# anzeA/Tarok

Hardware: AMD Instinct MI355X
Metric: env steps/sec at 65 536 parallel 4-player games; 1/2/4/8 MI355X (higher is better)
Workload: dtype u64

## Files before the change

include/tarok_env.h:

```cpp
#ifndef TAROK_ENV_H
#define TAROK_ENV_H
#include <stdint.h>

#ifdef __cplusplus
extern "C" {
#endif

#define TAROK_ABI_VERSION 5
#define TAROK_MAX_CARDS_PER_LAUNCH 192
#define TAROK_GAMES_AHEAD 14

#define TAROK_OK 0
#define TAROK_EINVAL (-1)
#define TAROK_EHIP (-2)
#define TAROK_ENOMEM (-3)
#define TAROK_ENODEV (-4)

#define TAROK_MIX_ALL 0
#define TAROK_MIX_NAVADNA3 1
#define TAROK_MIX_BOT 2
#define TAROK_MIX_FIXED 16

#define TAROK_DEFER_EXCHANGE 1
#define TAROK_AUTO_RESET 2
// ... 133 lines not shown

int tarok_learn_returns_gae(tarok_env *env, int T, const uint8_t *done, const int16_t *reward, const uint64_t *obs,
                            const float *logp, const float *value, const uint8_t *action, float reward_scale, float gamma,
                            float lambda, float *rec_out, float *stats_out, float *scratch, void *stream);

int tarok_learn_returns_seats(tarok_env *env, int T, const uint8_t *done, const int16_t *reward, const uint64_t *obs,
                              const float *logp, const float *value, const uint8_t *action, float reward_scale, int gae,
                              float gamma, float lambda, int seats, const uint8_t *seats_per_game, float *rec_out,
                              float *stats_out, float *scratch, void *stream);

#define TAROK_LEARN_SELECT_TILE 2048
int64_t tarok_learn_select_scratch_bytes(int64_t M);
int tarok_learn_select(tarok_env *env, int64_t M, const float *rec, int64_t *index_out, int64_t *count_out,
                       void *scratch, void *stream);

int tarok_learn_chain(tarok_env *env, int64_t B, const uint64_t *feature_words, const int64_t *index, const float *rec,
                      const float *stats, float clip, float vf_coef, float ent_coef, const void *w1, const float *b1,
                      const void *w2, const float *b2, const void *w3, const float *b3, const void *w3t, const void *w2t,
                      uint64_t *Xw, void *H1, void *H2, void *dOut, void *dH2, void *dH1, float *scratch, float *terms_out,
                      float *running, void *stream);

int64_t tarok_learn_workspace_bytes(tarok_env *env);
int tarok_learn_dw(tarok_env *env, int64_t B, const uint64_t *Xw, const void *H1,
                   const void *H2, const void *dOut, const void *dH2, const void *dH1, const float *terms,
                   void *workspace, float *grad_out, void *stream);

int tarok_learn_adam(tarok_env *env, float *param, const float *grad, float *m, float *v, int32_t *step, float lr,
                     float beta1, float beta2, float eps, float max_norm, void *w1, void *w2, void *w3, void *w3t,
                     void *w2t, float *gnorm_out, int apply, void *stream);

int tarok_debug_stamps(tarok_env *env, uint64_t *stamps);
int tarok_debug_stamps_sized(tarok_env *env, uint64_t *stamps, int64_t n_words);
int tarok_debug_refill_selftest(tarok_env *env, int kind, int per_slot, uint32_t episode0, int order, int reps, uint64_t *report_out);

int tarok_get_state(tarok_env *env, uint64_t *lanes_out, void *stream);
int tarok_set_state(tarok_env *env, const uint64_t *lanes_in, void *stream);
int tarok_get_counters(tarok_env *env, uint32_t *episode_out, int32_t *score_sum_out, void *stream);

#ifdef __cplusplus
}
#endif
#endif
```

tarok_amd/_native.py:

```python
import ctypes as C
import os
import subprocess

HERE = os.path.dirname(os.path.abspath(__file__))
ROOT = os.path.dirname(HERE)
SRC = os.path.join(HERE, "csrc", "tarok_env.hip")
DEPS = [SRC, os.path.join(HERE, "csrc", "tarok_device.h"), os.path.join(HERE, "csrc", "deal_network.inc"),
        os.path.join(HERE, "csrc", "tarok_learner.inc"),
        os.path.join(ROOT, "include", "tarok_env.h")]
LIB_PATH = os.path.join(HERE, "libtarokenv.so")
ARCH = "gfx950"
COMPILE_FLAGS = ["--offload-arch=" + ARCH, "-O3", "-std=c++17", "-mllvm", "-amdgpu-kernarg-preload-count=16",
                 "-I", os.path.join(ROOT, "include")]

SYMBOLS = [
    "tarok_strerror", "tarok_abi_version", "tarok_device_count", "tarok_last_hip_error",
    "tarok_create", "tarok_destroy", "tarok_num_games", "tarok_set_option", "tarok_reset", "tarok_exchange",
    "tarok_legal_actions", "tarok_step", "tarok_prefetch", "tarok_policy_random", "tarok_step_random",
    "tarok_run_random", "tarok_krog_random", "tarok_rollout_random", "tarok_get_state", "tarok_set_state", "tarok_get_counters", "tarok_debug_stamps", "tarok_debug_stamps_sized", "tarok_debug_refill_selftest", "tarok_observe", "tarok_sample_policy", "tarok_policy_mlp", "tarok_policy_step", "tarok_policy_step_seats", "tarok_policy_step_versus", "tarok_expand_features", "tarok_ppo_loss",
    "tarok_targets_ref", "tarok_learn_returns", "tarok_learn_returns_gae", "tarok_learn_returns_seats", "tarok_learn_select_scratch_bytes", "tarok_learn_select",
    "tarok_learn_chain", "tarok_learn_workspace_bytes", "tarok_learn_dw", "tarok_learn_adam",
    "tarok_observe_ref", "tarok_observe_exchange_ref", "tarok_observe_hands_ref", "tarok_get_history", "tarok_set_history",
]


class TarokNativeError(RuntimeError):
    pass


def hipcc_path():
    for p in (os.environ.get("HIPCC"), "/opt/rocm/bin/hipcc"):
        if p and os.path.exists(p):
            return p
    return "hipcc"


def needs_build():
    if not os.path.exists(LIB_PATH):
        return True
    t = os.path.getmtime(LIB_PATH)
    return any(os.path.getmtime(d) > t for d in DEPS)


def build(force=False, verbose=False):
    if not force and not needs_build():
        return LIB_PATH
    import fcntl
    with open(LIB_PATH + ".lock", "w") as lock:
        fcntl.flock(lock, fcntl.LOCK_EX)
        try:
            if force or needs_build():
                tmp = "%s.tmp.%d" % (LIB_PATH, os.getpid())
# ... 61 lines not shown
    L.tarok_step_random.restype = i32; L.tarok_step_random.argtypes = [vp, vp, vp, vp, vp, vp, i32, vp]
    L.tarok_run_random.restype = i32; L.tarok_run_random.argtypes = [vp, i64, i32, i32, i32, vp, vp, vp, vp, i32, vp]
    L.tarok_krog_random.restype = i32; L.tarok_krog_random.argtypes = [vp, i32, i64, vp, vp, vp, vp, vp, i32, vp]
    L.tarok_rollout_random.restype = i32; L.tarok_rollout_random.argtypes = [vp, u32, vp, vp, vp, vp, vp, vp]
    L.tarok_get_state.restype = i32; L.tarok_get_state.argtypes = [vp, vp, vp]
    L.tarok_observe.restype = i32; L.tarok_observe.argtypes = [vp, vp, vp]
    L.tarok_sample_policy.restype = i32; L.tarok_sample_policy.argtypes = [vp, vp, vp, vp, vp, vp]
    L.tarok_policy_mlp.restype = i32; L.tarok_policy_mlp.argtypes = [vp] * 14
    L.tarok_policy_step.restype = i32; L.tarok_policy_step.argtypes = [vp] * 16 + [i32, vp]
    L.tarok_policy_step_seats.restype = i32; L.tarok_policy_step_seats.argtypes = [vp, i32, vp] + [vp] * 15 + [i32, vp]
    L.tarok_policy_step_versus.restype = i32; L.tarok_policy_step_versus.argtypes = [vp, i32, vp] + [vp] * 21 + [i32, vp]
    L.tarok_expand_features.restype = i32; L.tarok_expand_features.argtypes = [vp, i64, vp, vp, vp, vp]
    f32 = C.c_float
    L.tarok_ppo_loss.restype = i32; L.tarok_ppo_loss.argtypes = [vp, i64] + [vp] * 7 + [f32] * 3 + [vp] * 4
    L.tarok_targets_ref.restype = i32; L.tarok_targets_ref.argtypes = [vp, i32] + [vp] * 6 + [f32] + [vp] * 3
    L.tarok_learn_returns.restype = i32; L.tarok_learn_returns.argtypes = [vp, i32] + [vp] * 6 + [f32] + [vp] * 4
    L.tarok_learn_returns_gae.restype = i32; L.tarok_learn_returns_gae.argtypes = [vp, i32] + [vp] * 6 + [f32] * 3 + [vp] * 4
    L.tarok_learn_returns_seats.restype = i32
    L.tarok_learn_returns_seats.argtypes = [vp, i32] + [vp] * 6 + [f32, i32, f32, f32, i32] + [vp] * 5
    L.tarok_learn_select_scratch_bytes.restype = i64; L.tarok_learn_select_scratch_bytes.argtypes = [i64]
    L.tarok_learn_select.restype = i32; L.tarok_learn_select.argtypes = [vp, i64] + [vp] * 5
    L.tarok_learn_chain.restype = i32; L.tarok_learn_chain.argtypes = [vp, i64] + [vp] * 4 + [f32] * 3 + [vp] * 18
    L.tarok_learn_workspace_bytes.restype = i64; L.tarok_learn_workspace_bytes.argtypes = [vp]
    L.tarok_learn_dw.restype = i32; L.tarok_learn_dw.argtypes = [vp, i64] + [vp] * 10
    L.tarok_learn_adam.restype = i32; L.tarok_learn_adam.argtypes = [vp] * 6 + [f32] * 5 + [vp] * 6 + [i32, vp]
    L.tarok_observe_ref.restype = i32; L.tarok_observe_ref.argtypes = [vp, vp, vp, vp]
    L.tarok_observe_exchange_ref.restype = i32; L.tarok_observe_exchange_ref.argtypes = [vp, vp, vp]
    L.tarok_observe_hands_ref.restype = i32; L.tarok_observe_hands_ref.argtypes = [vp, vp, vp]
    L.tarok_get_history.restype = i32; L.tarok_get_history.argtypes = [vp, vp, vp]
    L.tarok_set_history.restype = i32; L.tarok_set_history.argtypes = [vp, vp, vp]
    L.tarok_debug_stamps.restype = i32; L.tarok_debug_stamps.argtypes = [vp, vp]
    L.tarok_debug_stamps_sized.restype = i32; L.tarok_debug_stamps_sized.argtypes = [vp, vp, i64]
    L.tarok_debug_refill_selftest.restype = i32; L.tarok_debug_refill_selftest.argtypes = [vp, i32, i32, u32, i32, i32, vp]
    L.tarok_set_state.restype = i32; L.tarok_set_state.argtypes = [vp, vp, vp]
    L.tarok_get_counters.restype = i32; L.tarok_get_counters.argtypes = [vp, vp, vp, vp]
    _lib = L
    return L


def check(code):
    if code != 0:
        L = lib()
        raise TarokNativeError("libtarokenv: %s (code %d, hipError %d)" % (
            L.tarok_strerror(code).decode(), code, L.tarok_last_hip_error()))
```

tarok_amd/csrc/tarok_device.h:

```cpp
#pragma once
#include <hip/hip_runtime.h>
#include <stdint.h>

typedef unsigned long long u64;
typedef uint32_t u32;

#define TK_VGPR_BUDGET(B) __attribute__((amdgpu_num_vgpr((B) - 1)))
#define TK_KERNEL(threads, B) __global__ __launch_bounds__(threads) TK_VGPR_BUDGET(B)
#define TK_VGPR_STR2(x) #x
#define TK_VGPR_STR(x) TK_VGPR_STR2(x)
#define TK_VGPR_TOP(B, TOP)                                                                                           \
    do {                                                                                                              \
        static_assert((B) % 8 == 0 && (B) <= 256 && (TOP) == (B) - 1, "TK_VGPR_TOP(B, B - 1), B a multiple of 8");     \
        asm volatile("" ::: "v" TK_VGPR_STR(TOP));                                                                    \
    } while (0)

#define TK_BIT(i) (1ULL << (i))
#define TK_DECK ((1ULL << 54) - 1)
#define TK_TAROK (((1ULL << 22) - 1) << 32)
#define TK_PAGAT TK_BIT(32)
#define TK_V5 (TK_BIT(7) | TK_BIT(15) | TK_BIT(23) | TK_BIT(31) | TK_BIT(32) | TK_BIT(52) | TK_BIT(53))
#define TK_V4 (TK_BIT(6) | TK_BIT(14) | TK_BIT(22) | TK_BIT(30))
#define TK_V3 (TK_BIT(5) | TK_BIT(13) | TK_BIT(21) | TK_BIT(29))
#define TK_V2 (TK_BIT(4) | TK_BIT(12) | TK_BIT(20) | TK_BIT(28))
// ... 22 lines not shown
    g.C = x0 & TK_DECK; g.A = y0 & TK_DECK; g.B = y1 & TK_DECK;
    u32 m0 = (u32)(x0 >> 54), m2 = (u32)(y0 >> 54), m3 = (u32)(y1 >> 54);
    g.nt = 0; g.leader = (m0 >> 2) & 3; g.trick_no = (m0 >> 4) & 15; g.phase = m0 >> 8;
    g.talon = x1 & ((1ULL << 36) - 1);
    g.trick = 0;
    g.tl = (u32)(x1 >> 60) & 7; g.error = (u32)(x1 >> 63);
    g.contract = m2 & 15; g.declarer = (m2 >> 4) & 3; g.king = (m2 >> 6) & 3;
    g.team = m3 & 15; g.epar = (m3 >> 4) & 15; g.cprev = 0;
}

__device__ __forceinline__ void pack_play(const Game &g, u64 &x0, u64 &x1) {
    x0 = g.C | ((u64)(g.nt | (g.leader << 2) | (g.trick_no << 4) | (g.phase << 8)) << 54);
    x1 = g.talon | ((u64)g.trick << 36) | ((u64)g.tl << 60) | ((u64)g.error << 63);
}
__device__ __forceinline__ void pack_seats(const Game &g, u64 &y0, u64 &y1) {
    y0 = g.A | ((u64)(g.contract | (g.declarer << 4) | (g.king << 6) | ((g.cprev >> 2) << 8)) << 54);
    y1 = g.B | ((u64)(g.team | (g.epar << 4) | ((g.cprev & 3) << 8)) << 54);
}
__device__ __forceinline__ void pack(const Game &g, u64 &x0, u64 &x1, u64 &y0, u64 &y1) {
    pack_play(g, x0, x1);
    pack_seats(g, y0, y1);
}

__device__ __forceinline__ int popc64(u64 m) { return __popcll(m); }

template <class F> constexpr u32 tk_tt(F f) { return f(0xF0u, 0xCCu, 0xAAu) & 0xFFu; }
#define TK_BITOP3(a, b, c, ...) ((u32)__builtin_amdgcn_bitop3_b32((a), (b), (c), tk_tt([](u32 a_, u32 b_, u32 c_) { return (__VA_ARGS__); })))
#define TK_LO(x) ((u32)(x))
#define TK_HI(x) ((u32)((x) >> 32))
#ifndef TK_KEEP_VGPR
#define TK_KEEP_VGPR(x) asm volatile("" : "+v"(x))
#endif
#define TK_U64(lo, hi) (((u64)(u32)(hi) << 32) | (u64)(u32)(lo))

__device__ __forceinline__ u64 seat_cards(const Game &g, u32 s) {
    u64 a = (s & 1) ? g.A : ~g.A, b = (s & 2) ? g.B : ~g.B;
    return a & b & TK_DECK;
}
#define TK_C_PAD (0xFFC00000ULL << 32)
template <bool C_PADDED = false>
__device__ __forceinline__ u64 hand_of(const Game &g, u32 s) {
    u32 ma = (u32)((int)(s << 31) >> 31), mb = (u32)((int)(s << 30) >> 31);
    u32 tl = TK_BITOP3(TK_LO(g.A), ma, TK_LO(g.C), ~c_ & ~(a_ ^ b_));
    u32 th = TK_BITOP3(TK_HI(g.A), ma, TK_HI(g.C), ~c_ & ~(a_ ^ b_));
    u32 hl = TK_BITOP3(tl, TK_LO(g.B), mb, a_ & ~(b_ ^ c_));
    u32 hh = TK_BITOP3(th, TK_HI(g.B), mb, a_ & ~(b_ ^ c_));
    if (!C_PADDED) hh &= 0x3FFFFFu;
    return TK_U64(hl, hh);
}
template <int S> __device__ __forceinline__ u64 pile_of(const Game &g) {
    u32 l, h;
    if (S == 0)      { l = TK_BITOP3(TK_LO(g.A), TK_LO(g.B), TK_LO(g.C), ~a_ & ~b_ & c_); h = TK_BITOP3(TK_HI(g.A), TK_HI(g.B), TK_HI(g.C), ~a_ & ~b_ & c_); }
    else if (S == 1) { l = TK_BITOP3(TK_LO(g.A), TK_LO(g.B), TK_LO(g.C), a_ & ~b_ & c_);  h = TK_BITOP3(TK_HI(g.A), TK_HI(g.B), TK_HI(g.C), a_ & ~b_ & c_); }
    else if (S == 2) { l = TK_BITOP3(TK_LO(g.A), TK_LO(g.B), TK_LO(g.C), ~a_ & b_ & c_);  h = TK_BITOP3(TK_HI(g.A), TK_HI(g.B), TK_HI(g.C), ~a_ & b_ & c_); }
    else             { l = TK_BITOP3(TK_LO(g.A), TK_LO(g.B), TK_LO(g.C), a_ & b_ & c_);   h = TK_BITOP3(TK_HI(g.A), TK_HI(g.B), TK_HI(g.C), a_ & b_ & c_); }
    return TK_U64(l, h);
}

__device__ __forceinline__ u64 ids_mask(u64 ids, int first, int n) {
    u64 m = 0;
#pragma unroll
    for (int i = 0; i < 6; i++)
        if (i >= first && i < first + n) m |= 1ULL << ((ids >> (6 * i)) & 63);
    return m;
}
__device__ __forceinline__ u64 talon_all(const Game &g) { return ids_mask(g.talon, 0, 6); }
// ... 424 lines not shown
```

tarok_amd/csrc/tarok_env.hip:

```cpp
#include "tarok_device.h"

#include <hip/hip_runtime.h>
#include <stddef.h>
#include <stdint.h>
#include <stdio.h>
#include <stdlib.h>
#include <string.h>
#include <type_traits>
#include <utility>

#include "../../include/tarok_env.h"

#define TK_BLOCK 256
#define TK_PF_SLOTS (4 * TK_BLOCK)
#define TK_GRAPH_CACHE 16
#define TK_REFILL_CAP (TK_BLOCK * TK_AHEAD)
#define TK_REFILL_FAN 8
#define TK_RC(group, k) ((((size_t)(group)) * 4 + (k)) * 32)
#define TK_BULK_EVERY 32u
#define TK_BULK_CAP ((TK_BULK_EVERY / 4) * TK_BLOCK)

#define TK_AHEAD TAROK_GAMES_AHEAD
#define TK_LINE(episode) ((u32)(episode) % (u32)TK_AHEAD)
#define TK_FINQ 128
#define TK_STREAM_STORE(ptr, val) __builtin_nontemporal_store((val), (ptr))
#define TK_WAIT_LOADS() __builtin_amdgcn_s_waitcnt(0x0F70)
#define TK_RARE(c) __builtin_expect(!!(c), 0)
#define TK_USUAL(c) __builtin_expect(!!(c), 1)

struct __attribute__((aligned(64))) AuxLine {
    ulonglong2 n01, n23; u64 nkey; u32 nep;
    u32 pad[5];
};
struct __attribute__((aligned(64))) Aux { AuxLine line[TK_AHEAD]; };
static_assert(sizeof(AuxLine) == 64 && sizeof(Aux) == 64 * TK_AHEAD, "64 bytes per next-game line");
static_assert((TK_BLOCK * sizeof(Aux)) % 128 == 0, "a play group's next-game lines end on an L2 line boundary");
static_assert(TK_AHEAD >= 2 && TK_AHEAD <= 15, "epar / cprev are 4-bit fields");
struct __attribute__((aligned(32))) Counters {
    int4 score_sum;
    u32 episode;
    u32 pad[3];
};
static_assert(sizeof(Counters) == 32, "Counters is half a cache line");

struct tarok_env {
    int device;
    int64_t n;
    u64 offset, seed;
    int mix, flags;
    ulonglong2 *s01, *s23;
    Aux *aux;
    Counters *cnt;
    uint16_t *nstale;
    u64 *gkey;
    uint8_t *hist;
    u64 *rlist;
    u32 *rcount;
    u64 *elist;
    u32 *epoch;
// ... 286 lines not shown
            lists = elist; cap = TK_BULK_CAP;
#pragma unroll
            for (u32 q = 0; q < TK_REFILL_FAN; q++) {
                bool has = q < fan && g0 + q < play_groups;
                cum[q + 1] = cum[q] + (has ? min(tk_ld(&rcount[TK_RC(g0 + q, 2 + which)]), (u32)TK_BULK_CAP) : 0u);
            }
        }
        for (u32 j = tid; j < cum[TK_REFILL_FAN]; j += nthreads) {
            u32 q = 0;
#pragma unroll
            for (u32 r = 1; r < TK_REFILL_FAN; r++) q += j >= cum[r] ? 1u : 0u;
            u32 base = 0;
#pragma unroll
            for (u32 r = 0; r < TK_REFILL_FAN; r++) base = (r == q) ? cum[r] : base;
            u64 en = tk_ld(&lists[((int64_t)(g0 + q) * 2 + which) * cap + (j - base)]);
            deal_into_buffer(aux, (int64_t)(g0 + q) * TK_BLOCK + (u32)(en & 0xFFFF), (u32)(en >> 32), seed, offset, mix);
        }
    }
    if (any || bulk) {
        __syncthreads();
        if (any && tid < fan && g0 + tid < play_groups) rcount[TK_RC(g0 + tid, par ^ 1u)] = 0u;
        if (bulk && tid < fan && g0 + tid < play_groups) rcount[TK_RC(g0 + tid, 2 + which)] = 0u;
    }
}

template <bool HIST>
__device__ __forceinline__ void play_role(
    u32 group, u32 tid,
    int64_t n, u64 seed, u64 offset, int mix, int flags, int cards, int64_t stride, TkCount count, u32 *epoch, u32 play_groups, u32 fan,
    uint8_t *__restrict__ action_out, int16_t *__restrict__ reward,
    uint8_t *__restrict__ done, uint16_t *__restrict__ trick, u64 *__restrict__ obs, uint8_t *__restrict__ hist,
    ulonglong2 *__restrict__ s01, ulonglong2 *__restrict__ s23, Aux *aux, Counters *__restrict__ cnt,
    u64 *__restrict__ gkey, u64 *rlist, u32 *rcount, u64 *__restrict__ stamps) {
    __shared__ unsigned short push_list[TK_REFILL_CAP];
    __shared__ u32 push_ep[TK_BLOCK];
    __shared__ u32 push_count;
    __shared__ u32 finq[TK_BLOCK / 64][9][TK_FINQ];
    __shared__ int sacc[4][TK_BLOCK];
    if (tid == 0) push_count = 0;
    sacc[0][tid] = 0; sacc[1][tid] = 0; sacc[2][tid] = 0; sacc[3][tid] = 0;
    __syncthreads();
    u32 fq_head = 0, fq_n = 0;
    u32 (*fq)[TK_FINQ] = finq[tid >> 6];
    auto drain_finished = [&](u32 cnt_) __attribute__((always_inline)) {
        u32 lane = tid & 63;
        if (lane < cnt_) {
            u32 e = (fq_head + lane) & (TK_FINQ - 1);
            Game f;
            f.A = TK_U64(fq[0][e], fq[1][e]); f.B = TK_U64(fq[2][e], fq[3][e]); f.C = TK_U64(fq[4][e], fq[5][e] & 0x3FFFFFu);
            u32 m = fq[7][e], ri = fq[8][e];
            f.talon = TK_U64(fq[6][e], (m >> 24) & 15u);
            f.contract = m & 15; f.declarer = (m >> 4) & 3; f.king = (m >> 6) & 3; f.team = (m >> 8) & 15;
            f.tl = (m >> 12) & 7; f.trick_no = (m >> 16) & 15; f.leader = (m >> 20) & 3;
            f.trick = 0; f.nt = 0; f.phase = TK_PHASE_DONE; f.error = 0; f.epar = 0; f.cprev = 0;
            u64 sc = final_scores(f);
            u32 t = ri & 0xFFFFu;
            if (reward) {
                u64 rs = sc;
                if ((flags & TAROK_REWARD_REF) && (f.contract == TK_BERAC || f.contract == TK_ODPRTI_BERAC)) {
                    int dv = f.trick_no >= 12 ? -20 : 20;
                    u32 d = f.declarer;
                    rs = pack_scores(d == 0 ? (int)(int16_t)(sc & 0xFFFF) : dv, d == 1 ? (int)(int16_t)((sc >> 16) & 0xFFFF) : dv,
                                     d == 2 ? (int)(int16_t)((sc >> 32) & 0xFFFF) : dv, d == 3 ? (int)(int16_t)(sc >> 48) : dv);
                }
                reinterpret_cast<u64 *>(reward)[(int64_t)group * TK_BLOCK + t + (int64_t)(ri >> 16) * stride] = rs;
            }
            atomicAdd(&sacc[0][t], (int)(int16_t)(sc & 0xFFFF)); atomicAdd(&sacc[1][t], (int)(int16_t)((sc >> 16) & 0xFFFF));
            atomicAdd(&sacc[2][t], (int)(int16_t)((sc >> 32) & 0xFFFF)); atomicAdd(&sacc[3][t], (int)(int16_t)(sc >> 48));
        }
        fq_head = (fq_head + cnt_) & (TK_FINQ - 1);
        fq_n -= cnt_;
    };
    u64 t_real0 = 0, t_cyc0 = 0, t_play = 0;
    if (stamps) { t_real0 = __builtin_amdgcn_s_memrealtime(); t_cyc0 = __builtin_amdgcn_s_memtime(); }
    int64_t i = (int64_t)group * TK_BLOCK + tid;
    bool valid = i < n;
    int64_t ic = valid ? i : n - 1;
    Game g;
    load_game(g, s01, s23, ic);
    u64 key = gkey[ic];
    bool autoreset = (flags & TAROK_AUTO_RESET) != 0;
    bool berac = g.contract == TK_BERAC || g.contract == TK_ODPRTI_BERAC;
    bool spec = valid && ((g.phase == TK_PHASE_PLAY && (int)g.nt + cards >= 4 &&
                           (berac || (int)(g.trick_no * 4 + g.nt) + cards >= 48)) ||
                          g.phase == TK_PHASE_DONE);
    u32 cprev0 = valid ? g.cprev : 0u;
    u32 allowed = TK_AHEAD - min(cprev0, (u32)TK_AHEAD);
    int4 acc = make_int4(0, 0, 0, 0);
    u32 cur_ep = 0;
    ulonglong2 na = make_ulonglong2(0, 0), nb = na, na2 = na, nb2 = na;
    u64 nkey = 0, nkey2 = 0;
    u32 nep1 = 0, nep2 = 0;
    bool ok1 = false, ok2 = false;
    auto line_tag = [&](bool &ok, u32 &nep, u32 tag) __attribute__((always_inline)) { nep = tag; ok = true; };
    static_assert(offsetof(AuxLine, nkey) == 32 && offsetof(AuxLine, nep) == 40, "key and tag share the line's third 16 bytes");
    auto load_line = [&](const AuxLine *ln, ulonglong2 &a, ulonglong2 &b, u64 &k, bool &ok, u32 &nep) __attribute__((always_inline)) {
        a = ln->n01; b = ln->n23;
        uint3 kt = *reinterpret_cast<const uint3 *>(__builtin_assume_aligned(&ln->nkey, 16));
        k = TK_U64(kt.x, kt.y);
        line_tag(ok, nep, kt.z);
    };
    const bool all_play = autoreset && __ballot(valid && g.phase == TK_PHASE_PLAY) == ~0ULL;
    const bool aligned = all_play && (cards & 3) == 0 && __ballot(g.nt != 0) == 0;
    if (spec) {
        acc = cnt[i].score_sum;
        cur_ep = cnt[i].episode;
        if (autoreset && allowed > 0) {
            load_line(&aux[i].line[TK_LINE(g.epar + 1)], na, nb, nkey, ok1, nep1);
            if (!aligned && allowed > 1 && cards > 4)
                load_line(&aux[i].line[TK_LINE(g.epar + 2)], na2, nb2, nkey2, ok2, nep2);
        }
    }
    TK_WAIT_LOADS();
    u32 par = launch_phase<1>(count, play_groups, fan) & 1u;
    launch_counted<1>(epoch);
    g.cprev = 0;
    u32 consumed = 0;
    bool resync = false;
    bool blocked = false;
    bool acc_dirty = false, seats_dirty = false, touched = false;
    u64 legal = (valid && g.phase == TK_PHASE_PLAY) ? legal_now(g) : 0;
    u64 c_lead = 0;
    u32 legal_hi = 0;
    u32 rctr = 0, ocar = 0;
    u32 resync_v = 0;
    u32 lim = spec ? allowed : 0u;
    auto fetch_lines = [&](bool lacks, bool lacks2) __attribute__((always_inline)) {
        if (lacks) load_line(&aux[i].line[TK_LINE(cur_ep + 1)], na, nb, nkey, ok1, nep1);
        if (lacks2) load_line(&aux[i].line[TK_LINE(cur_ep + 2)], na2, nb2, nkey2, ok2, nep2);
    };
    auto play_card = [&](auto all_tag, auto nt_tag, auto std_tag, int64_t row, int ci) __attribute__((always_inline)) {
        constexpr bool ALL = decltype(all_tag)::value;
        constexpr int NT = decltype(nt_tag)::value;
        constexpr bool STD = decltype(std_tag)::value;
        if constexpr (NT >= 0) g.nt = (u32)NT;
        constexpr bool TOP_UP_EARLY = ALL && NT == 0;
        constexpr bool TOP_UP_LATE = !(ALL && NT == 3);
        if constexpr (TOP_UP_EARLY) {
            if (nep1 != cur_ep + 1 && consumed < lim) {
                u32 off = g.epar + 1 >= (u32)TK_AHEAD ? 0u : (g.epar + 1) * (u32)sizeof(AuxLine);
                load_line(reinterpret_cast<const AuxLine *>(reinterpret_cast<const char *>(aux[i].line) + off), na, nb, nkey, ok1, nep1);
            }
        }
        const bool v = ALL ? true : valid;
// ... 109 lines not shown
                        TK_WAIT_LOADS();
                    }
                }
                bool swap = renew && !blocked && ok1 && nep1 == cur_ep + 1;
                if (swap) {
                    swap_in();
                    ok1 = ok2 && consumed + 1 < allowed;
                    ok2 = false;
                }
                bool deal_here = renew && !swap;
                if (deal_here && consumed < allowed) resync = true;
                if (deal_here) blocked = true;
                deal_in_place(deal_here, g, key);
                if (renew) { cur_ep++; consumed++; seats_dirty = true; }
            }
        }
        if constexpr (ALIGNED && NT < 3) legal = legal_mask_follow(hand_of<true>(g, (g.leader + g.nt) & 3), g.trick & 63, g.contract, legal_hi);
        else if constexpr (ALIGNED) legal = legal_mask(hand_of<true>(g, g.leader), false, 0u, g.contract);
        else legal = (ALL || (v && g.phase == TK_PHASE_PLAY)) ? legal_now(g) : 0;
        if (v) {
            const u32 fin01 = ALL ? (u32)res : (fin ? 1u : 0u);
            if constexpr (ALIGNED) {
                if constexpr (NT < 3) ocar += TK_OBS_CARD;
                else ocar = obs_carry(g.leader, g.trick_no << 2);
                TK_STREAM_STORE(&obs[row], obs_word_with(ocar, g.error, fin01, legal));
            } else {
                TK_STREAM_STORE(&obs[row], obs_word_with<true>(g, false, legal) | ((u64)(ALL ? fin01 : ((fin || g.phase == TK_PHASE_DONE) ? 1u : 0u)) << 62));
            }
            if (STD || done) TK_STREAM_STORE(&done[row], (uint8_t)fin01);
        }
    };
    int64_t row = i;
    typedef std::integral_constant<int, -1> nt_any;
    if (all_play) {
        if (aligned) {
            auto tricks = [&](auto std_tag) __attribute__((always_inline)) {
                touched = true; seats_dirty = true;
                g.C |= TK_C_PAD;
                rctr = rng_ctr(128u + g.trick_no * 4).v;
                ocar = obs_carry(g.leader, g.trick_no << 2);
                for (int c = 0; c < cards; c += 4) {
                    play_card(std::true_type{}, std::integral_constant<int, 0>{}, std_tag, row, c); row += stride;
                    play_card(std::true_type{}, std::integral_constant<int, 1>{}, std_tag, row, c + 1); row += stride;
                    play_card(std::true_type{}, std::integral_constant<int, 2>{}, std_tag, row, c + 2); row += stride;
                    play_card(std::true_type{}, std::integral_constant<int, 3>{}, std_tag, row, c + 3); row += stride;
                }
                g.C &= TK_DECK;
            };
            if (action_out && done && !trick) tricks(std::true_type{});
            else tricks(std::false_type{});
        } else {
            for (int c = 0; c < cards; c++, row += stride) play_card(std::true_type{}, nt_any{}, std::false_type{}, row, c);
        }
    } else {
        for (int c = 0; c < cards; c++, row += stride) play_card(std::false_type{}, nt_any{}, std::false_type{}, row, c);
    }
    while (fq_n) drain_finished(min(fq_n, 64u));
    __builtin_amdgcn_s_waitcnt(0xC07F);
    {
        int4 sa = make_int4(sacc[0][tid], sacc[1][tid], sacc[2][tid], sacc[3][tid]);
        if (sa.x | sa.y | sa.z | sa.w) { acc.x += sa.x; acc.y += sa.y; acc.z += sa.z; acc.w += sa.w; acc_dirty = true; }
    }
    u32 np = (resync || resync_v != 0) ? (u32)TK_AHEAD : min(consumed, (u32)TK_AHEAD);
    if (valid) {
        g.cprev = np;
        if (acc_dirty) cnt[i].score_sum = acc;
        if (consumed) { cnt[i].episode = cur_ep; gkey[i] = key; }
        if (touched || consumed || cprev0 != np) store_game(g, s01, s23, i, seats_dirty || cprev0 != np);
    }
    if (stamps) t_play = __builtin_amdgcn_s_memtime() - t_cyc0;
    if (valid && np) {
        u32 pos = atomicAdd(&push_count, np);
        push_ep[tid] = cur_ep;
        for (u32 j = 0; j < np; j++) push_list[pos + j] = (unsigned short)(j * TK_BLOCK + tid);
    }
    __syncthreads();
    u32 total = push_count;
    u64 *lst = rlist + ((int64_t)group * 2 + par) * TK_REFILL_CAP;
    for (u32 j = tid; j < total; j += TK_BLOCK) {
        u32 en = push_list[j], t = en % TK_BLOCK;
        lst[j] = ((u64)(push_ep[t] + TK_AHEAD - en / TK_BLOCK) << 32) | t;
    }
    if (tid == 0) rcount[TK_RC(group, par)] = total;
    if (stamps && (tid & 63) == 0) {
        u64 w = (u64)i >> 6;
        stamps[3 * w + 0] = t_real0;
        stamps[3 * w + 1] = __builtin_amdgcn_s_memrealtime();
        stamps[3 * w + 2] = ((__builtin_amdgcn_s_memtime() - t_cyc0) << 32) | (t_play & 0xFFFFFFFFULL);
    }
}

#define TK_PLAY_ARGS                                                                                                             \
    int64_t n, u64 seed, u64 offset, int mix, int flags, int cards, int64_t stride, u32 play_groups, u32 *epoch, u32 fan,         \
        uint8_t *__restrict__ action_out, int16_t *__restrict__ reward,                                                           \
        uint8_t *__restrict__ done, uint16_t *__restrict__ trick, u64 *__restrict__ obs, uint8_t *__restrict__ hist,              \
        ulonglong2 *__restrict__ s01, ulonglong2 *__restrict__ s23, Aux *aux, Counters *__restrict__ cnt,                         \
        u64 *__restrict__ gkey, u64 *rlist, u32 *rcount, u64 *__restrict__ stamps
template <bool HIST>
TK_KERNEL(TK_BLOCK, 168) __attribute__((amdgpu_waves_per_eu(3, 3))) void k_play_wide(TK_PLAY_ARGS) {
    TK_VGPR_TOP(168, 167);
    TkCount count = launch_count<1>(epoch, play_groups);
    if (blockIdx.x >= play_groups)
        refill_role<false>(blockIdx.x - play_groups, threadIdx.x, TK_BLOCK, seed, offset, mix, play_groups, count, epoch, fan, false, aux, rlist, rcount, nullptr);
    else {
        play_role<HIST>(blockIdx.x, threadIdx.x, n, seed, offset, mix, flags, cards, stride, count, epoch, play_groups, fan,
                        action_out, reward, done, trick, obs, hist, s01, s23, aux, cnt, gkey, rlist, rcount, stamps);
    }
}

__device__ __forceinline__ void deal_in_place_wave(bool deal_here, Game &gd, u64 &kd, u64 seed, u64 offset, int64_t i, u32 ep, int mix) {
    u64 pend = __ballot(deal_here);
    if (pend == 0) return;
    u64 dkey = 0;
    if (deal_here) dkey = game_key(seed, offset + (u64)i, ep);
    u64 h0 = 0, h1 = 0, h2 = 0, h3 = 0, tal = 0;
    u32 lane = __lane_id();
    while (pend) {
        int l = __builtin_ctzll(pend);
        pend &= pend - 1;
        u32 klo = (u32)__builtin_amdgcn_readlane((int)(u32)dkey, l);
        u32 khi = (u32)__builtin_amdgcn_readlane((int)(u32)(dkey >> 32), l);
// ... 1399 lines not shown
    if (!e || !obs_out) return TAROK_EINVAL;
    HIPCHK(hipSetDevice(e->device));
    hipLaunchKernelGGL(k_legal, grid_for(e->n), dim3(TK_BLOCK), 0, (hipStream_t)stream, e->n, e->s01, e->s23,
                       (u64 *)obs_out, seat_out);
    HIPCHK(hipGetLastError());
    return TAROK_OK;
}

static inline u64 *stamps_for(const tarok_env *e, size_t words) { return (e->stamps && e->stamps_words >= words) ? e->stamps : nullptr; }

static inline void launch_play(tarok_env *e, bool random, int cards, int64_t stride, const uint8_t *action_in,
                               uint8_t *action_out, int16_t *reward, uint8_t *done, uint16_t *trick, uint64_t *obs,
                               int flags, hipStream_t s) {
    u32 groups = (u32)((e->n + TK_BLOCK - 1) / TK_BLOCK);
    u32 fan = e->refill_fan;
    dim3 grid(groups + (groups + fan - 1) / fan);
    e->launched = 1;
    if (cards == 1 && e->lazy_refill) grid = dim3(groups);
    if (cards == 1) {
#define TK_LAUNCH_STEP(R, Z)                                                                                             \
    hipLaunchKernelGGL((k_step<R, Z>), grid, dim3(TK_BLOCK), 0, s, e->n, e->seed, e->offset, e->mix, flags, groups, e->epoch, \
                       fan, action_in, action_out, reward, done, trick, (u64 *)obs, e->hist, e->s01, e->s23, e->aux, e->cnt,  \
                       e->gkey, e->rlist, e->rcount, e->elist)
        if (e->lazy_refill) { if (random) TK_LAUNCH_STEP(true, true); else TK_LAUNCH_STEP(false, true); }
        else                { if (random) TK_LAUNCH_STEP(true, false); else TK_LAUNCH_STEP(false, false); }
#undef TK_LAUNCH_STEP
        return;
    }
#define TK_LAUNCH_PLAY(H)                                                                                              \
    hipLaunchKernelGGL((k_play_wide<H>), grid, dim3(TK_BLOCK), 0, s, e->n, e->seed, e->offset, e->mix, flags, cards, stride, \
                       groups, e->epoch, fan, action_out, reward, done, trick, (u64 *)obs, e->hist, e->s01,            \
                       e->s23, e->aux, e->cnt, e->gkey, e->rlist, e->rcount, stamps)
    u64 *stamps = stamps_for(e, 3 * (size_t)((e->n + 63) / 64));
    if (e->hist) TK_LAUNCH_PLAY(true); else TK_LAUNCH_PLAY(false);
#undef TK_LAUNCH_PLAY
}

int tarok_step(tarok_env *e, const uint8_t *action, int16_t *reward_out, uint8_t *done_out, uint16_t *trick_out,
               uint64_t *obs_out, int flags, void *stream) {
    if (!e || !action || !obs_out) return TAROK_EINVAL;
    HIPCHK(hipSetDevice(e->device));
    launch_play(e, false, 1, e->n, action, nullptr, reward_out, done_out, trick_out, obs_out, flags, (hipStream_t)stream);
    HIPCHK(hipGetLastError());
    return TAROK_OK;
}

static inline void launch_policy(tarok_env *e, const uint64_t *obs, uint8_t *action, hipStream_t s) {
    if (e->n >= (1 << 21) && (((uintptr_t)obs & 15) | ((uintptr_t)action & 1)) == 0)
        hipLaunchKernelGGL(k_policy_x4, dim3((unsigned)((e->n + 4 * TK_BLOCK - 1) / (4 * TK_BLOCK))), dim3(TK_BLOCK), 0, s, e->n,
                           (const u64 *)obs, e->gkey, action);
    else
        hipLaunchKernelGGL(k_policy, grid_for(e->n), dim3(TK_BLOCK), 0, s, e->n, (const u64 *)obs, e->gkey, action);
}

int tarok_policy_random(tarok_env *e, const uint64_t *obs, uint8_t *action_out, void *stream) {
    if (!e || !obs || !action_out) return TAROK_EINVAL;
    HIPCHK(hipSetDevice(e->device));
    launch_policy(e, obs, action_out, (hipStream_t)stream);
    HIPCHK(hipGetLastError());
    return TAROK_OK;
}

int tarok_step_random(tarok_env *e, uint8_t *action_out, int16_t *reward_out, uint8_t *done_out, uint16_t *trick_out,
                      uint64_t *obs_out, int flags, void *stream) {
    if (!e || !obs_out) return TAROK_EINVAL;
    HIPCHK(hipSetDevice(e->device));
// ... 102 lines not shown
    void *buf = nullptr;
    unsigned long long *rep = nullptr;
    HIPCHK(hipMalloc(&buf, rows * (size_t)n * (8 + 8 + 1 + 1) + 64));
    hipError_t r = hipMalloc((void **)&rep, 49 * sizeof(unsigned long long));
    if (r == hipSuccess) r = hipMemset(rep, 0, 49 * sizeof(unsigned long long));
    if (r != hipSuccess) { (void)hipFree(buf); g_last_hip = (int)r; return TAROK_EHIP; }
    uint64_t *obs = (uint64_t *)buf;
    int16_t *reward = (int16_t *)(obs + rows * n);
    uint8_t *action = (uint8_t *)(reward + rows * n * 4), *done = action + rows * n;
    u32 groups = (u32)((n + TK_BLOCK - 1) / TK_BLOCK);
    for (int it = 0; it < reps; it++) {
        hipLaunchKernelGGL(k_dbg_clear_lines, grid_for(n), dim3(TK_BLOCK), 0, 0, e->aux, n);
        hipLaunchKernelGGL(k_dbg_fill_lists, dim3(groups), dim3(TK_BLOCK), 0, 0, e->rlist, e->rcount, n, (u32)per_slot, episode0, (u32)order);
        if (kind == 0) launch_play(e, true, 1, n, nullptr, action, reward, done, nullptr, obs, TAROK_AUTO_RESET, 0);
        else if (kind == 1) {
            hipLaunchKernelGGL(k_legal, grid_for(n), dim3(TK_BLOCK), 0, 0, n, e->s01, e->s23, (u64 *)obs, (int8_t *)nullptr);
            launch_policy(e, obs, action, 0);
            launch_play(e, false, 1, n, action, nullptr, reward, done, nullptr, obs, TAROK_AUTO_RESET, 0);
        } else launch_play(e, true, kind == 2 ? 4 : 2, n, nullptr, action, reward, done, nullptr, obs, TAROK_AUTO_RESET, 0);
        hipLaunchKernelGGL(k_dbg_check_lines, grid_for(n), dim3(TK_BLOCK), 0, 0, e->aux, n, e->seed, e->offset, e->mix, (u32)per_slot, episode0, rep);
    }
    r = hipDeviceSynchronize();
    if (r == hipSuccess) r = hipMemcpy(report_out, rep, 49 * sizeof(unsigned long long), hipMemcpyDeviceToHost);
    if (r == hipSuccess) r = hipMemset(e->rcount, 0, TK_RC(groups, 0) * sizeof(u32));
    if (r == hipSuccess) {
        hipLaunchKernelGGL(k_dbg_clear_lines, grid_for(n), dim3(TK_BLOCK), 0, 0, e->aux, n);
        r = hipDeviceSynchronize();
    }
    (void)hipFree(buf); (void)hipFree(rep);
    if (r != hipSuccess) { g_last_hip = (int)r; return TAROK_EHIP; }
    return TAROK_OK;
}

int tarok_observe(tarok_env *e, void *features_out, void *stream) {
    if (!e || !features_out) return TAROK_EINVAL;
    HIPCHK(hipSetDevice(e->device));
    hipLaunchKernelGGL(k_observe, grid_for(e->n), dim3(TK_BLOCK), 0, (hipStream_t)stream, e->n, e->s01, e->s23,
                       (uint2 *)features_out);
    HIPCHK(hipGetLastError());
    return TAROK_OK;
}

int tarok_observe_ref(tarok_env *e, uint8_t *record_out, int32_t *meta_out, void *stream) {
    if (!e || !record_out) return TAROK_EINVAL;
    if (!e->hist) return TAROK_EINVAL;
    HIPCHK(hipSetDevice(e->device));
    hipLaunchKernelGGL(k_observe_ref, dim3((unsigned)((e->n + OR_GAMES - 1) / OR_GAMES)), dim3(256), 0, (hipStream_t)stream, e->n,
                       e->s01, e->s23, e->hist, (uint4 *)record_out, (int4 *)meta_out);
    HIPCHK(hipGetLastError());
    return TAROK_OK;
}

int tarok_observe_exchange_ref(tarok_env *e, uint8_t *out, void *stream) {
    if (!e || !out) return TAROK_EINVAL;
    HIPCHK(hipSetDevice(e->device));
    hipLaunchKernelGGL(k_observe_exchange_ref, grid_for(e->n), dim3(TK_BLOCK), 0, (hipStream_t)stream, e->n, e->s01, e->s23,
                       (uint2 *)out);
    HIPCHK(hipGetLastError());
    return TAROK_OK;
}

int tarok_observe_hands_ref(tarok_env *e, uint8_t *out, void *stream) {
    if (!e || !out) return TAROK_EINVAL;
    HIPCHK(hipSetDevice(e->device));
    hipLaunchKernelGGL(k_observe_hands_ref, grid_for(e->n), dim3(TK_BLOCK), 0, (hipStream_t)stream, e->n, e->s01, e->s23,
                       (uint2 *)out);
// ... 308 lines not shown
```

tarok_amd/env.py:

```python
import ctypes as C

import numpy as np
import torch

from . import _native
from . import karte as K


def _u64(t):
    return t.detach().cpu().numpy().view(np.uint64)


class Obs:

    def __init__(self, words):
        self.words = words

    @property
    def mask(self):
        return self.words & K.OBS_MASK

    @property
    def seat(self):
        return (self.words >> K.OBS_SEAT_SHIFT) & 3
# ... 22 lines not shown
            raise _native.TarokNativeError("TarokVecEnv needs an MI355X: no GPU is visible and there is no CPU fallback")
        self.L = L
        self.n = int(n_games)
        self.device_index = int(device)
        self.device = torch.device("cuda", self.device_index)
        self.seed, self.mix, self.game_offset = int(seed), int(mix), int(game_offset)
        h = C.c_void_p()
        self.history = bool(history)
        _native.check(L.tarok_create(C.byref(h), self.device_index, self.n, self.game_offset, self.seed, self.mix,
                                     K.HISTORY if history else 0))
        self._h = h
        self.set_option(refill_fan, lazy_refill)
        with torch.cuda.device(self.device):
            self.obs_words = torch.zeros(self.n, dtype=torch.int64, device=self.device)
            self.reward = torch.zeros((self.n, 4), dtype=torch.int16, device=self.device)
            self.done = torch.zeros(self.n, dtype=torch.uint8, device=self.device)
            self.action = torch.full((self.n,), 255, dtype=torch.uint8, device=self.device)
            self.trick = None

    def set_option(self, refill_fan=None, lazy_refill=None):
        if refill_fan is not None:
            _native.check(self.L.tarok_set_option(self._h, K.OPT_REFILL_FAN, int(refill_fan)))
        if lazy_refill is not None:
            _native.check(self.L.tarok_set_option(self._h, K.OPT_LAZY_REFILL, int(lazy_refill)))

    def refill_selftest(self, kind, per_slot, episode0=100, order=0, reps=1):
        import numpy as np
        rep = np.zeros(49, np.uint64)
        with torch.cuda.device(self.device):
            torch.cuda.synchronize(self.device)
            _native.check(self.L.tarok_debug_refill_selftest(self._h, int(kind), int(per_slot), int(episode0), int(order), int(reps),
                                                             rep.ctypes.data))
        return int(rep[0]), rep[1:].reshape(8, 6)[: min(8, int(rep[0]))]

    def close(self):
        if self._h is not None:
            torch.cuda.synchronize(self.device)
            self.L.tarok_destroy(self._h)
            self._h = None

    def __del__(self):
        try:
            self.close()
        except Exception:
            pass

    def _stream(self):
        return C.c_void_p(torch.cuda.current_stream(self.device).cuda_stream)

    def _dev(self, x, dtype, shape):
        if x is None:
            return None
        t = torch.as_tensor(x)
        t = t.to(device=self.device, dtype=dtype).contiguous()
        if tuple(t.shape) != tuple(shape):
            raise ValueError("expected shape %s, got %s" % (tuple(shape), tuple(t.shape)))
        return t

    @staticmethod
    def _p(t):
        return None if t is None else C.c_void_p(t.data_ptr())

    def reset(self, episode=0, deals=None, contract=None, declarer=None, king_suit=None,
              talon_choice=None, discards=None, defer_exchange=False, clear_counters=True):
        n = self.n
        deals = self._dev(deals, torch.uint8, (n, 54))
# ... 360 lines not shown
```

Before: 196.0 billion.

## Build refill lists with wave ballots instead of shared-memory atomics

Replaces the shared-memory atomicAdd push list in the play kernel with per-wave bit-sliced ballots and mbcnt prefix counts. Each thread now writes its refill entries directly to global memory at a computed offset. This removes the shared atomic, the shared push arrays and the second pass that translated them. It also hoists the state and counter loads ahead of the first barrier, skips line prefetch on the aligned path, and adds optional edge timing stamps plus a debug API to dump refill lists. Entry order within a group changes from atomic order to a deterministic per-wave order.

```diff
diff --git a/include/tarok_env.h b/include/tarok_env.h
--- a/include/tarok_env.h
+++ b/include/tarok_env.h
@@ -189,6 +189,7 @@
 int tarok_debug_stamps(tarok_env *env, uint64_t *stamps);
 int tarok_debug_stamps_sized(tarok_env *env, uint64_t *stamps, int64_t n_words);
 int tarok_debug_refill_selftest(tarok_env *env, int kind, int per_slot, uint32_t episode0, int order, int reps, uint64_t *report_out);
+int tarok_debug_refill_lists(tarok_env *env, uint32_t *counts_out, uint64_t *entries_out, uint8_t *redealt_out);
 
 int tarok_get_state(tarok_env *env, uint64_t *lanes_out, void *stream);
 int tarok_set_state(tarok_env *env, const uint64_t *lanes_in, void *stream);
diff --git a/tarok_amd/_native.py b/tarok_amd/_native.py
--- a/tarok_amd/_native.py
+++ b/tarok_amd/_native.py
@@ -17,7 +17,7 @@
     "tarok_strerror", "tarok_abi_version", "tarok_device_count", "tarok_last_hip_error",
     "tarok_create", "tarok_destroy", "tarok_num_games", "tarok_set_option", "tarok_reset", "tarok_exchange",
     "tarok_legal_actions", "tarok_step", "tarok_prefetch", "tarok_policy_random", "tarok_step_random",
-    "tarok_run_random", "tarok_krog_random", "tarok_rollout_random", "tarok_get_state", "tarok_set_state", "tarok_get_counters", "tarok_debug_stamps", "tarok_debug_stamps_sized", "tarok_debug_refill_selftest", "tarok_observe", "tarok_sample_policy", "tarok_policy_mlp", "tarok_policy_step", "tarok_policy_step_seats", "tarok_policy_step_versus", "tarok_expand_features", "tarok_ppo_loss",
+    "tarok_run_random", "tarok_krog_random", "tarok_rollout_random", "tarok_get_state", "tarok_set_state", "tarok_get_counters", "tarok_debug_stamps", "tarok_debug_stamps_sized", "tarok_debug_refill_selftest", "tarok_debug_refill_lists", "tarok_observe", "tarok_sample_policy", "tarok_policy_mlp", "tarok_policy_step", "tarok_policy_step_seats", "tarok_policy_step_versus", "tarok_expand_features", "tarok_ppo_loss",
     "tarok_targets_ref", "tarok_learn_returns", "tarok_learn_returns_gae", "tarok_learn_returns_seats", "tarok_learn_select_scratch_bytes", "tarok_learn_select",
     "tarok_learn_chain", "tarok_learn_workspace_bytes", "tarok_learn_dw", "tarok_learn_adam",
     "tarok_observe_ref", "tarok_observe_exchange_ref", "tarok_observe_hands_ref", "tarok_get_history", "tarok_set_history",
@@ -145,6 +145,7 @@
     L.tarok_debug_stamps.restype = i32; L.tarok_debug_stamps.argtypes = [vp, vp]
     L.tarok_debug_stamps_sized.restype = i32; L.tarok_debug_stamps_sized.argtypes = [vp, vp, i64]
     L.tarok_debug_refill_selftest.restype = i32; L.tarok_debug_refill_selftest.argtypes = [vp, i32, i32, u32, i32, i32, vp]
+    L.tarok_debug_refill_lists.restype = i32; L.tarok_debug_refill_lists.argtypes = [vp, vp, vp, vp]
     L.tarok_set_state.restype = i32; L.tarok_set_state.argtypes = [vp, vp, vp]
     L.tarok_get_counters.restype = i32; L.tarok_get_counters.argtypes = [vp, vp, vp, vp]
     _lib = L
diff --git a/tarok_amd/csrc/tarok_device.h b/tarok_amd/csrc/tarok_device.h
--- a/tarok_amd/csrc/tarok_device.h
+++ b/tarok_amd/csrc/tarok_device.h
@@ -78,6 +78,28 @@
 #define TK_KEEP_VGPR(x) asm volatile("" : "+v"(x))
 #endif
 #define TK_U64(lo, hi) (((u64)(u32)(hi) << 32) | (u64)(u32)(lo))
+
+#if defined(__HIPCC__) || defined(TK_EMULATED_MBCNT)
+struct TkListVotes { u64 b[4]; };
+__device__ __forceinline__ TkListVotes tk_list_votes(u32 np) {
+    TkListVotes v;
+    v.b[0] = __ballot((np & 1u) != 0); v.b[1] = __ballot((np & 2u) != 0);
+    v.b[2] = __ballot((np & 4u) != 0); v.b[3] = __ballot((np & 8u) != 0);
+    return v;
+}
+__device__ __forceinline__ u32 tk_votes_below(u64 vote) {
+    return __builtin_amdgcn_mbcnt_hi(TK_HI(vote), __builtin_amdgcn_mbcnt_lo(TK_LO(vote), 0u));
+}
+__device__ __forceinline__ u32 tk_list_below(const TkListVotes &v) {
+    return tk_votes_below(v.b[0]) + 2u * tk_votes_below(v.b[1]) + 4u * tk_votes_below(v.b[2]) + 8u * tk_votes_below(v.b[3]);
+}
+__device__ __forceinline__ u32 tk_list_total(const TkListVotes &v) {
+    return (u32)__popcll(v.b[0]) + 2u * (u32)__popcll(v.b[1]) + 4u * (u32)__popcll(v.b[2]) + 8u * (u32)__popcll(v.b[3]);
+}
+__device__ __forceinline__ u32 tk_list_base(u32 tot0, u32 tot1, u32 tot2, u32 wave) {
+    return (wave > 0 ? tot0 : 0u) + (wave > 1 ? tot1 : 0u) + (wave > 2 ? tot2 : 0u);
+}
+#endif
 
 __device__ __forceinline__ u64 seat_cards(const Game &g, u32 s) {
     u64 a = (s & 1) ? g.A : ~g.A, b = (s & 2) ? g.B : ~g.B;
diff --git a/tarok_amd/csrc/tarok_env.hip b/tarok_amd/csrc/tarok_env.hip
--- a/tarok_amd/csrc/tarok_env.hip
+++ b/tarok_amd/csrc/tarok_env.hip
@@ -25,6 +25,7 @@
 #define TK_FINQ 128
 #define TK_STREAM_STORE(ptr, val) __builtin_nontemporal_store((val), (ptr))
 #define TK_WAIT_LOADS() __builtin_amdgcn_s_waitcnt(0x0F70)
+#define TK_FLAG_EDGE_STAMPS (1 << 30)
 #define TK_RARE(c) __builtin_expect(!!(c), 0)
 #define TK_USUAL(c) __builtin_expect(!!(c), 1)
 
@@ -377,14 +378,27 @@
     uint8_t *__restrict__ done, uint16_t *__restrict__ trick, u64 *__restrict__ obs, uint8_t *__restrict__ hist,
     ulonglong2 *__restrict__ s01, ulonglong2 *__restrict__ s23, Aux *aux, Counters *__restrict__ cnt,
     u64 *__restrict__ gkey, u64 *rlist, u32 *rcount, u64 *__restrict__ stamps) {
-    __shared__ unsigned short push_list[TK_REFILL_CAP];
-    __shared__ u32 push_ep[TK_BLOCK];
-    __shared__ u32 push_count;
+    __shared__ u32 push_total[TK_BLOCK / 64];
     __shared__ u32 finq[TK_BLOCK / 64][9][TK_FINQ];
     __shared__ int sacc[4][TK_BLOCK];
-    if (tid == 0) push_count = 0;
+    u64 t_real0 = 0, t_cyc0 = 0, t_play = 0, t_edges = 0;
+    if (stamps) { t_real0 = __builtin_amdgcn_s_memrealtime(); t_cyc0 = __builtin_amdgcn_s_memtime(); }
+    int64_t i = (int64_t)group * TK_BLOCK + tid;
+    bool valid = i < n;
+    int64_t ic = valid ? i : n - 1;
+    const ulonglong2 raw01 = s01[ic], raw23 = s23[ic];
+    u64 key = gkey[ic];
+    int4 acc = make_int4(0, 0, 0, 0);
+    u32 cur_ep = 0;
+    if (valid) {
+        acc = cnt[i].score_sum;
+        cur_ep = cnt[i].episode;
+    }
     sacc[0][tid] = 0; sacc[1][tid] = 0; sacc[2][tid] = 0; sacc[3][tid] = 0;
     __syncthreads();
+    __builtin_amdgcn_sched_barrier(0);
+    Game g;
+    unpack(g, raw01.x, raw01.y, raw23.x, raw23.y);
     u32 fq_head = 0, fq_n = 0;
     u32 (*fq)[TK_FINQ] = finq[tid >> 6];
     auto drain_finished = [&](u32 cnt_) __attribute__((always_inline)) {
@@ -416,14 +430,6 @@
         fq_head = (fq_head + cnt_) & (TK_FINQ - 1);
         fq_n -= cnt_;
     };
-    u64 t_real0 = 0, t_cyc0 = 0, t_play = 0;
-    if (stamps) { t_real0 = __builtin_amdgcn_s_memrealtime(); t_cyc0 = __builtin_amdgcn_s_memtime(); }
-    int64_t i = (int64_t)group * TK_BLOCK + tid;
-    bool valid = i < n;
-    int64_t ic = valid ? i : n - 1;
-    Game g;
-    load_game(g, s01, s23, ic);
-    u64 key = gkey[ic];
     bool autoreset = (flags & TAROK_AUTO_RESET) != 0;
     bool berac = g.contract == TK_BERAC || g.contract == TK_ODPRTI_BERAC;
     bool spec = valid && ((g.phase == TK_PHASE_PLAY && (int)g.nt + cards >= 4 &&
@@ -431,8 +437,6 @@
                           g.phase == TK_PHASE_DONE);
     u32 cprev0 = valid ? g.cprev : 0u;
     u32 allowed = TK_AHEAD - min(cprev0, (u32)TK_AHEAD);
-    int4 acc = make_int4(0, 0, 0, 0);
-    u32 cur_ep = 0;
     ulonglong2 na = make_ulonglong2(0, 0), nb = na, na2 = na, nb2 = na;
     u64 nkey = 0, nkey2 = 0;
     u32 nep1 = 0, nep2 = 0;
@@ -447,14 +451,11 @@
     };
     const bool all_play = autoreset && __ballot(valid && g.phase == TK_PHASE_PLAY) == ~0ULL;
     const bool aligned = all_play && (cards & 3) == 0 && __ballot(g.nt != 0) == 0;
-    if (spec) {
-        acc = cnt[i].score_sum;
-        cur_ep = cnt[i].episode;
-        if (autoreset && allowed > 0) {
-            load_line(&aux[i].line[TK_LINE(g.epar + 1)], na, nb, nkey, ok1, nep1);
-            if (!aligned && allowed > 1 && cards > 4)
-                load_line(&aux[i].line[TK_LINE(g.epar + 2)], na2, nb2, nkey2, ok2, nep2);
-        }
+    if (aligned) nep1 = cur_ep;
+    else if (spec && autoreset && allowed > 0) {
+        load_line(&aux[i].line[TK_LINE(g.epar + 1)], na, nb, nkey, ok1, nep1);
+        if (allowed > 1 && cards > 4)
+            load_line(&aux[i].line[TK_LINE(g.epar + 2)], na2, nb2, nkey2, ok2, nep2);
     }
     TK_WAIT_LOADS();
     u32 par = launch_phase<1>(count, play_groups, fan) & 1u;
@@ -630,6 +631,7 @@
     };
     int64_t row = i;
     typedef std::integral_constant<int, -1> nt_any;
+    if (stamps) t_edges = (__builtin_amdgcn_s_memtime() - t_cyc0) & 0xFFFFFFFFULL;
     if (all_play) {
         if (aligned) {
             auto tricks = [&](auto std_tag) __attribute__((always_inline)) {
@@ -653,6 +655,7 @@
     } else {
         for (int c = 0; c < cards; c++, row += stride) play_card(std::false_type{}, nt_any{}, std::false_type{}, row, c);
     }
+    if (stamps) t_edges |= (__builtin_amdgcn_s_memtime() - t_cyc0) << 32;
     while (fq_n) drain_finished(min(fq_n, 64u));
     __builtin_amdgcn_s_waitcnt(0xC07F);
     {
@@ -667,24 +670,33 @@
         if (touched || consumed || cprev0 != np) store_game(g, s01, s23, i, seats_dirty || cprev0 != np);
     }
     if (stamps) t_play = __builtin_amdgcn_s_memtime() - t_cyc0;
-    if (valid && np) {
-        u32 pos = atomicAdd(&push_count, np);
-        push_ep[tid] = cur_ep;
-        for (u32 j = 0; j < np; j++) push_list[pos + j] = (unsigned short)(j * TK_BLOCK + tid);
-    }
+    if (!valid) np = 0;
+    const TkListVotes votes = tk_list_votes(np);
+    if ((tid & 63) == 0) push_total[tid >> 6] = tk_list_total(votes);
     __syncthreads();
-    u32 total = push_count;
-    u64 *lst = rlist + ((int64_t)group * 2 + par) * TK_REFILL_CAP;
-    for (u32 j = tid; j < total; j += TK_BLOCK) {
-        u32 en = push_list[j], t = en % TK_BLOCK;
-        lst[j] = ((u64)(push_ep[t] + TK_AHEAD - en / TK_BLOCK) << 32) | t;
-    }
-    if (tid == 0) rcount[TK_RC(group, par)] = total;
+    const u32 wave = tid >> 6;
+    const u32 tot0 = push_total[0], tot1 = push_total[1], tot2 = push_total[2], tot3 = push_total[3];
+    u64 *lst = rlist + ((int64_t)group * 2 + par) * TK_REFILL_CAP + tk_list_base(tot0, tot1, tot2, wave) + tk_list_below(votes);
+    {
+        u32 ep = cur_ep + TK_AHEAD;
+        auto entries = [&](auto count_tag) __attribute__((always_inline)) {
+            constexpr u32 COUNT = decltype(count_tag)::value;
+#pragma unroll
+            for (u32 j = 0; j < COUNT; j++) lst[j] = ((u64)(ep - j) << 32) | tid;
+            lst += COUNT; ep -= COUNT;
+        };
+        if (np & 8u) entries(std::integral_constant<u32, 8>{});
+        if (np & 4u) entries(std::integral_constant<u32, 4>{});
+        if (np & 2u) entries(std::integral_constant<u32, 2>{});
+        if (np & 1u) entries(std::integral_constant<u32, 1>{});
+    }
+    if (tid == 0) rcount[TK_RC(group, par)] = tot0 + tot1 + tot2 + tot3;
     if (stamps && (tid & 63) == 0) {
         u64 w = (u64)i >> 6;
         stamps[3 * w + 0] = t_real0;
         stamps[3 * w + 1] = __builtin_amdgcn_s_memrealtime();
         stamps[3 * w + 2] = ((__builtin_amdgcn_s_memtime() - t_cyc0) << 32) | (t_play & 0xFFFFFFFFULL);
+        if (flags & TK_FLAG_EDGE_STAMPS) stamps[3 * (u64)((n + 63) >> 6) + w] = t_edges;
     }
 }
 
@@ -2150,6 +2162,8 @@
                        groups, e->epoch, fan, action_out, reward, done, trick, (u64 *)obs, e->hist, e->s01,            \
                        e->s23, e->aux, e->cnt, e->gkey, e->rlist, e->rcount, stamps)
     u64 *stamps = stamps_for(e, 3 * (size_t)((e->n + 63) / 64));
+    flags &= ~TK_FLAG_EDGE_STAMPS;
+    if (stamps_for(e, 4 * (size_t)((e->n + 63) / 64))) flags |= TK_FLAG_EDGE_STAMPS;
     if (e->hist) TK_LAUNCH_PLAY(true); else TK_LAUNCH_PLAY(false);
 #undef TK_LAUNCH_PLAY
 }
@@ -2318,6 +2332,36 @@
     return TAROK_OK;
 }
 
+int tarok_debug_refill_lists(tarok_env *e, uint32_t *counts_out, uint64_t *entries_out, uint8_t *redealt_out) {
+    if (!e) return TAROK_EINVAL;
+    HIPCHK(hipSetDevice(e->device));
+    HIPCHK(hipDeviceSynchronize());
+    const size_t groups = (size_t)((e->n + TK_BLOCK - 1) / TK_BLOCK);
+    if (counts_out) {
+        u32 *rc = (u32 *)malloc(TK_RC(groups, 0) * sizeof(u32));
+        if (!rc) return TAROK_ENOMEM;
+        hipError_t r = hipMemcpy(rc, e->rcount, TK_RC(groups, 0) * sizeof(u32), hipMemcpyDeviceToHost);
+        if (r == hipSuccess)
+            for (size_t g = 0; g < groups; g++) { counts_out[2 * g] = rc[TK_RC(g, 0)]; counts_out[2 * g + 1] = rc[TK_RC(g, 1)]; }
+        free(rc);
+        HIPCHK(r);
+    }
+    if (entries_out) HIPCHK(hipMemcpy(entries_out, e->rlist, groups * 2 * TK_REFILL_CAP * sizeof(u64), hipMemcpyDeviceToHost));
+    if (redealt_out) {
+        ulonglong2 *seats = (ulonglong2 *)malloc((size_t)e->n * sizeof(ulonglong2));
+        if (!seats) return TAROK_ENOMEM;
+        hipError_t r = hipMemcpy(seats, e->s23, (size_t)e->n * sizeof(ulonglong2), hipMemcpyDeviceToHost);
+        if (r == hipSuccess)
+            for (int64_t i = 0; i < e->n; i++) {
+                u32 m2 = (u32)(seats[i].x >> 54), m3 = (u32)(seats[i].y >> 54);
+                redealt_out[i] = (uint8_t)(((m3 >> 8) & 3u) | (((m2 >> 8) & 3u) << 2));
+            }
+        free(seats);
+        HIPCHK(r);
+    }
+    return TAROK_OK;
+}
+
 int tarok_observe(tarok_env *e, void *features_out, void *stream) {
     if (!e || !features_out) return TAROK_EINVAL;
     HIPCHK(hipSetDevice(e->device));
diff --git a/tarok_amd/env.py b/tarok_amd/env.py
--- a/tarok_amd/env.py
+++ b/tarok_amd/env.py
@@ -78,6 +78,22 @@
             _native.check(self.L.tarok_debug_refill_selftest(self._h, int(kind), int(per_slot), int(episode0), int(order), int(reps),
                                                              rep.ctypes.data))
         return int(rep[0]), rep[1:].reshape(8, 6)[: min(8, int(rep[0]))]
+
+    def refill_lists(self):
+        import numpy as np
+        groups = (self.n + 255) // 256
+        cap = 256 * K.GAMES_AHEAD
+        counts = np.zeros((groups, 2), np.uint32)
+        entries = np.zeros((groups, 2, cap), np.uint64)
+        redealt = np.zeros(self.n, np.uint8)
+        with torch.cuda.device(self.device):
+            _native.check(self.L.tarok_debug_refill_lists(self._h, counts.ctypes.data, entries.ctypes.data, redealt.ctypes.data))
+        assert (counts <= cap).all()
+        lists = []
+        for g in range(groups):
+            en = np.concatenate([entries[g, p, :counts[g, p]] for p in range(2)])
+            lists.append(np.stack([(en >> np.uint64(32)).astype(np.int64), (en & np.uint64(0xFFFFFFFF)).astype(np.int64)], 1))
+        return lists, counts, redealt
 
     def close(self):
         if self._h is not None:
```

Measured after the change: 197.6 billion (median of 6 runs). Within noise of the previous version (+0.8%).
